# modular-ngp/phys-autodiff

Measured on NVIDIA B200. Metric: grid points/sec, fused MLP + finite-difference physics loss, higher is better.
Workload: dtype f32

## Files before the change

### phys_autodiff_b200/csrc/capi.cu

```cuda
#include "../../include/physad_b200.h"
#include "deep_data_kernels.cuh"
#include "deep_grad_kernels.cuh"
#include "deep_kernels.cuh"
#include "deep_tangent_kernels.cuh"
#include "deep_tc_kernels.cuh"
#include "dense_kernels.cuh"
#include "grad_kernels.cuh"
#include "stage_kernels.cuh"
#include "tangent_grad_kernels.cuh"
#include "tangent_kernels.cuh"

#include <algorithm>
#include <cmath>
#include <cstdio>
#include <cstdlib>
#include <cstring>
#include <string>
#include <unordered_map>
#include <vector>

using namespace physad;

namespace {

// ... 208 lines not shown
                    if (out) out->push_back(t * nzl + (nzl - rem));
                    continue;
                }
                const int take = std::max(1, std::min(rem, int(space)));
                cur += seg_cost + take;
                rem -= take;
                open = true;
                if (cur + seg_cost + 1.0 > cap) {
                    ++blocks; cur = 0.0; open = false;
                    if (out) out->push_back(t * nzl + (nzl - rem));
                }
            }
        }
        if (open) { ++blocks; if (out) out->push_back(tiles * nzl); }
        return blocks;
    };
    double lo = 1.0 + seg_cost, hi = double(tiles) * (nzl + seg_cost) + 1.0;
    for (int it = 0; it < 60; ++it) {
        const double mid = 0.5 * (lo + hi);
        if (fill(mid, nullptr) <= slots) hi = mid; else lo = mid;
    }
    std::vector<int> r;
    fill(hi, &r);
    return r;
}

int build_fused_plan(physad_ctx* c, const physad_grid* g, const physad_slab& s, int TX, int TY, long long slots,
                     cudaStream_t st) {
    if (int rc = ensure_coord_tables(c, g, st)) return rc;
    auto& p = c->plan;
    p.cxs = c->tab.dev;
    p.cys = p.cxs + g->nx;
    p.czs = p.cys + g->ny;
    const int key[10] = {g->nx, g->ny, g->nz, s.z_begin, s.z_end, c->cfg.norm, TX, TY, int(slots), 1};
    if (std::memcmp(key, p.key, sizeof(key)) == 0) return 0;
    const int tiles = ((g->nx + TX - 1) / TX) * ((g->ny + TY - 1) / TY), nzl = s.z_end - s.z_begin;
    const long long want = std::min<long long>(slots, (long long)tiles * nzl);
    const std::vector<int> ranges = balanced_ranges(tiles, nzl, want, 0.9);
    const size_t bytes = ranges.size() * sizeof(int);
    if (bytes > p.cap) {
        if (p.dev) CU(cudaFree(p.dev));
        p.dev = nullptr; p.cap = 0;
        CU(cudaMalloc(&p.dev, bytes));
        p.cap = bytes;
    }
    CU(cudaMemcpyAsync(p.dev, ranges.data(), bytes, cudaMemcpyHostToDevice, st));
    CU(cudaStreamSynchronize(st));
    p.ranges = reinterpret_cast<const int*>(p.dev);
    p.blocks = int(ranges.size()) - 1;
    std::memcpy(p.key, key, sizeof(key));
    return 0;
}

template <int H, int P, int TYB, int UNROLL, int MINB, bool PACKED, bool SPLITBAR, bool DPRES>
int launch_fused_d(physad_ctx* c, const physad_grid* g, const physad_slab& s, const float tc[3], bool xchg, double* acc,
                   float* const R[4], cudaStream_t st, int blocks_per_sm_cap = 0) {
    constexpr int TX = 32, TY = TYB * P;
    auto kern = k_fused_mlp_phys_loss<H, P, TYB, UNROLL, MINB, PACKED, SPLITBAR, DPRES>;
    const size_t smem = size_t(4) * 4 * (TX + 2) * (TY + 2) * sizeof(float);
    static const long long env_blocks = getenv("PHYSAD_FUSED_BLOCKS") ? atoll(getenv("PHYSAD_FUSED_BLOCKS")) : 0;
    int& per_sm = c->blocks_per_sm[reinterpret_cast<const void*>(kern)];
    if (per_sm == 0) {
        CU(cudaFuncSetAttribute(kern, cudaFuncAttributeMaxDynamicSharedMemorySize, int(smem)));
        int q = 0;
        CU(cudaOccupancyMaxActiveBlocksPerMultiprocessor(&q, kern, 32 * TYB, smem));
        if (q < 1) return fail(PHYSAD_E_UNSUPPORTED, "fused kernel does not fit on an SM");
        per_sm = q;
    }
    const int tiles_x = (g->nx + TX - 1) / TX, tiles_y = (g->ny + TY - 1) / TY;
    const int bps = blocks_per_sm_cap > 0 ? std::min(per_sm, blocks_per_sm_cap) : per_sm;
    const long long slots = env_blocks > 0 ? env_blocks : (long long)bps * c->sm_count;
    if (int rc = build_fused_plan(c, g, s, TX, TY, slots, st)) return rc;
    const long long blocks = c->plan.blocks;
    FusedArgs a{};
    a.nx = g->nx; a.ny = g->ny; a.nz = g->nz;
    a.z_begin = s.z_begin; a.z_end = s.z_end;
    a.tiles_x = tiles_x; a.tiles_y = tiles_y;
    a.cxs = c->plan.cxs; a.cys = c->plan.cys; a.czs = c->plan.czs; a.ranges = c->plan.ranges;
    a.m1p1 = c->cfg.norm == 1; a.periodic = g->periodic != 0;
    a.inv2dt = inv2(g->dt); a.inv2hx = inv2(g->hx); a.inv2hy = inv2(g->hy); a.inv2hz = inv2(g->hz);
    a.inv2dt_d = inv2d(g->dt); a.inv2hx_d = inv2d(g->hx); a.inv2hy_d = inv2d(g->hy); a.inv2hz_d = inv2d(g->hz);
    if (int rc = ensure_partials(c, size_t(blocks))) return rc;
    a.partials = c->partials; a.ticket = c->ticket; a.acc_out = acc;
    for (int k = 0; k < 4; ++k) a.R[k] = R[k];
    if (xchg) {
        a.x.rank = c->xrank; a.x.world = c->xworld; a.x.epoch = c->xepoch + 1;
        for (int p = 0; p < XCHG_MAX_RANKS; ++p) a.x.peer[p] = c->xpeer[p];
    }
    a.status = c->d_status;
    if (c->want_host_seq) { a.host_res = c->d_res; a.host_seq = c->want_host_seq; }
    if (c->trace && blocks <= c->trace_blocks) a.trace = c->trace;
    MlpConst<H> k;
    fill_const<H>(c, tc, k);
    kern<<<unsigned(blocks), 32 * TYB, smem, st>>>(k, a);
    CU(cudaGetLastError());
    c->launches++;
    if (xchg) c->xepoch++;
    return 0;
}

template <int H, int P, int TYB, int UNROLL, int MINB, bool PACKED, bool SPLITBAR = false>
int launch_fused_t(physad_ctx* c, const physad_grid* g, const physad_slab& s, const float tc[3], bool xchg, double* acc,
                   float* const R[4], cudaStream_t st, int blocks_per_sm_cap = 0) {
    return launch_fused_d<H, P, TYB, UNROLL, MINB, PACKED, SPLITBAR, false>(c, g, s, tc, xchg, acc, R, st, blocks_per_sm_cap);
}

template <int H, bool DPRES>
int launch_fused_default(physad_ctx* c, const physad_grid* g, const physad_slab& s, const float tc[3], bool xchg,
                         double* acc, float* const R[4], cudaStream_t st) {
    const long long tile_planes = (long long)((g->nx + 31) / 32) * ((g->ny + 63) / 64) * (s.z_end - s.z_begin);
    if (tile_planes < 12LL * c->sm_count)
        return launch_fused_d<H, 4, 8, 2, 2, true, true, DPRES>(c, g, s, tc, xchg, acc, R, st, 1);
    return launch_fused_d<H, 4, 16, 2, 1, true, true, DPRES>(c, g, s, tc, xchg, acc, R, st, 0);
}

template <int H>
int launch_fused_h(physad_ctx* c, const physad_grid* g, const physad_slab& s, const float tc[3], bool dt, double* acc,
                   float* const R[4], cudaStream_t st) {
    if (c->exact_residuals) return launch_fused_default<H, true>(c, g, s, tc, dt, acc, R, st);
    switch (c->fused_variant) {
        default:
        case 0: return launch_fused_default<H, false>(c, g, s, tc, dt, acc, R, st);
        case 1: return launch_fused_t<H, 4, 8, 2, 2, true, true>(c, g, s, tc, dt, acc, R, st);
        case 2: return launch_fused_t<H, 4, 16, 2, 1, true, false>(c, g, s, tc, dt, acc, R, st);
        case 3: return launch_fused_t<H, 4, 8, 2, 1, false, false>(c, g, s, tc, dt, acc, R, st);
        case 4: return launch_fused_t<H, 2, 16, 4, 1, true, true>(c, g, s, tc, dt, acc, R, st);
        case 5: return launch_fused_t<H, 1, 8, 4, 4, true, false>(c, g, s, tc, dt, acc, R, st);
        case 6: return launch_fused_t<H, 2, 8, 2, 3, true, true>(c, g, s, tc, dt, acc, R, st);
        case 7: return launch_fused_t<H, 4, 8, 2, 2, true, true>(c, g, s, tc, dt, acc, R, st, 1);
    }
}

int launch_fused(physad_ctx* c, const physad_grid* g, const physad_slab& s, float t, float dt, double* acc,
                 float* const R[4], cudaStream_t st, bool xchg = false) {
    if (c->advection != 0)
        return fail(PHYSAD_E_UNSUPPORTED, "fused_loss: the fused kernel implements the reference's central scheme only; "
                                          "upwind advection runs stage-wise (generate_fields + phys_loss)");
    if (xchg && (c->xworld <= 1 || !c->xbuf))
        return fail(PHYSAD_E_INVALID, "fused_loss_allreduce: call physad_xchg_connect first");
    if (s.z_end == s.z_begin) {
        XchgArgs x{};
        if (xchg) {
            x.rank = c->xrank; x.world = c->xworld; x.epoch = c->xepoch + 1;
            for (int p = 0; p < XCHG_MAX_RANKS; ++p) x.peer[p] = c->xpeer[p];
        }
        k_xchg_only<<<1, 32, 0, st>>>(x, acc, c->want_host_seq ? c->d_res : nullptr, c->want_host_seq, c->d_status);
        CU(cudaGetLastError());
        c->launches++;
        if (xchg) c->xepoch++;
        return 0;
    }
    const float ts[3] = {t - dt, t, t + dt};
    const float tc[3] = {time_coord(ts[0], c->cfg.norm), time_coord(ts[1], c->cfg.norm), time_coord(ts[2], c->cfg.norm)};
    switch (template_h(c->cfg.H)) {
        case 32: return launch_fused_h<32>(c, g, s, tc, xchg, acc, R, st);
        case 64: return launch_fused_h<64>(c, g, s, tc, xchg, acc, R, st);
        case 128: return launch_fused_h<128>(c, g, s, tc, xchg, acc, R, st);
    }
    return fail(PHYSAD_E_UNSUPPORTED, "H > 128 not built");
}

template <int H, bool FIELDS>
int launch_grid_t(physad_ctx* c, const physad_grid* g, const physad_slab& s, const float tc[3], GridInferArgs a,
                  cudaStream_t st, int dtype = PHYSAD_F32) {
    const int nzl = s.z_end - s.z_begin;
    if (nzl == 0) return 0;
// ... 1945 lines not shown
```

### phys_autodiff_b200/csrc/fused_loss.cuh

```cuda
#pragma once
#include <type_traits>

#include "mlp_eval.cuh"

namespace physad {

constexpr int XCHG_MAX_RANKS = 8;

struct XSlot {
    double a, b;
    unsigned long long flag;
    unsigned long long pad;
};

struct XchgArgs {
    int rank, world;
    unsigned long long epoch;
    XSlot* peer[XCHG_MAX_RANKS];
};

__device__ __forceinline__ void st_release_sys(unsigned long long* p, unsigned long long v) {
    asm volatile("st.release.sys.global.u64 [%0], %1;" ::"l"(p), "l"(v) : "memory");
}
__device__ __forceinline__ unsigned long long ld_acquire_sys(const unsigned long long* p) {
// ... 1 lines not shown
    asm volatile("ld.acquire.sys.global.u64 %0, [%1];" : "=l"(v) : "l"(p) : "memory");
    return v;
}
__device__ __forceinline__ double ld_relaxed_sys(const double* p) {
    double v;
    asm volatile("ld.relaxed.sys.global.f64 %0, [%1];" : "=d"(v) : "l"(p) : "memory");
    return v;
}

__device__ __forceinline__ bool xchg_allreduce2(const XchgArgs& x, double& a, double& b) {
    const int lane = threadIdx.x & 31;
    const int set = int(x.epoch & 1ull) * XCHG_MAX_RANKS;
    bool ok = true;
    double pa = 0.0, pb = 0.0;
    if (lane < x.world) {
        XSlot* s = x.peer[lane] + set + x.rank;
        s->a = a;
        s->b = b;
        __threadfence_system();
        st_release_sys(&s->flag, x.epoch);
        const XSlot* r = x.peer[x.rank] + set + lane;
        const long long t0 = clock64();
        while (ld_acquire_sys(&r->flag) != x.epoch) {
            if (clock64() - t0 > 8000000000ll) { ok = false; break; }
            __nanosleep(64);
        }
        pa = ld_relaxed_sys(&r->a);
        pb = ld_relaxed_sys(&r->b);
    }
    ok = __all_sync(0xffffffffu, ok);
    double ta = 0.0, tb = 0.0;
    for (int p = 0; p < x.world; ++p) {
        ta += __shfl_sync(0xffffffffu, pa, p);
        tb += __shfl_sync(0xffffffffu, pb, p);
    }
    a = ok ? ta : __longlong_as_double(0x7ff8000000000000ll);
    b = ok ? tb : __longlong_as_double(0x7ff8000000000000ll);
    return ok;
}

struct HostResult {
    double a, b;
    unsigned long long status;
    unsigned long long seq;
};

struct ReduceSink {
    const XchgArgs* x = nullptr;
    HostResult* host = nullptr;
    unsigned long long host_seq = 0;
    unsigned int* status = nullptr;
};

constexpr int TRACE_SLOTS = 18;
__device__ __forceinline__ unsigned long long globaltimer_ns() {
    unsigned long long t;
    asm volatile("mov.u64 %0, %%globaltimer;" : "=l"(t));
    return t;
}
__device__ __forceinline__ unsigned int smid() {
    unsigned int r;
    asm volatile("mov.u32 %0, %%smid;" : "=r"(r));
    return r;
}

struct FusedArgs {
    int nx, ny, nz;
    int z_begin, z_end;
    int tiles_x, tiles_y;
    const float* cxs;
    const float* cys;
    const float* czs;
    const int* ranges;
    int m1p1, periodic;
    float inv2dt, inv2hx, inv2hy, inv2hz;
    double inv2dt_d, inv2hx_d, inv2hy_d, inv2hz_d;
    double2* partials;
    unsigned int* ticket;
    double* acc_out;
    float* R[4];
    XchgArgs x;
    HostResult* host_res;
    unsigned long long host_seq;
    unsigned int* status;
    unsigned long long* trace;
};

__device__ __forceinline__ double warp_sum(double v) {
#pragma unroll
    for (int o = 16; o > 0; o >>= 1) v += __shfl_xor_sync(0xffffffffu, v, o);
    return v;
}

template <int NWARPS>
__device__ __forceinline__ void grid_reduce2_lin(double a, double b, double2* partials, unsigned int* ticket, double* out,
                                                 double2* s_red, unsigned int* s_flag, unsigned int block_lin,
                                                 unsigned int nblocks, const ReduceSink* sink = nullptr) {
    const int lane = threadIdx.x & 31, wid = threadIdx.x >> 5;
    a = warp_sum(a);
    b = warp_sum(b);
    if (lane == 0) s_red[wid] = make_double2(a, b);
    __syncthreads();
    if (threadIdx.x == 0) {
        double sa = 0.0, sb = 0.0;
#pragma unroll
        for (int i = 0; i < NWARPS; ++i) { sa += s_red[i].x; sb += s_red[i].y; }
        partials[block_lin] = make_double2(sa, sb);
// ... 23 lines not shown
            out[0] = ta;
            out[1] = tb;
            *ticket = 0u;
            if (sink != nullptr) {
                if (!ok && sink->status) *sink->status = 1u;
                if (sink->host) {
                    sink->host->a = ta;
                    sink->host->b = tb;
                    sink->host->status = ok ? 0ull : 1ull;
                    __threadfence_system();
                    st_release_sys(&sink->host->seq, sink->host_seq);
                }
            }
        }
    }
}

template <int NWARPS>
__device__ __forceinline__ void grid_reduce2(double a, double b, double2* partials, unsigned int* ticket, double* out,
                                             double2* s_red, unsigned int* s_flag, const ReduceSink* sink = nullptr) {
    grid_reduce2_lin<NWARPS>(a, b, partials, ticket, out, s_red, s_flag, blockIdx.x, gridDim.x, sink);
}

static __global__ void k_xchg_only(const __grid_constant__ XchgArgs x, double* out, HostResult* host, unsigned long long host_seq,
                            unsigned int* status) {
    double a = 0.0, b = 0.0;
    const bool ok = xchg_allreduce2(x, a, b);
    if (threadIdx.x == 0) {
        out[0] = a; out[1] = b;
        if (!ok && status) *status = 1u;
        if (host) {
            host->a = a; host->b = b; host->status = ok ? 0ull : 1ull;
            __threadfence_system();
            st_release_sys(&host->seq, host_seq);
        }
    }
}

__device__ __forceinline__ unsigned smem_u32(const void* p) { return unsigned(__cvta_generic_to_shared(p)); }
__device__ __forceinline__ void mbar_init(unsigned long long* bar, unsigned count) {
    asm volatile("mbarrier.init.shared::cta.b64 [%0], %1;" ::"r"(smem_u32(bar)), "r"(count) : "memory");
}
__device__ __forceinline__ void mbar_arrive(unsigned long long* bar) {
    asm volatile("{ .reg .b64 st; mbarrier.arrive.shared::cta.b64 st, [%0]; }" ::"r"(smem_u32(bar)) : "memory");
}
__device__ __forceinline__ void mbar_wait(unsigned long long* bar, unsigned parity) {
    unsigned ok;
    do {
        asm volatile("{ .reg .pred p; mbarrier.try_wait.parity.shared::cta.b64 p, [%1], %2; selp.u32 %0, 1, 0, p; }"
                     : "=r"(ok) : "r"(smem_u32(bar)), "r"(parity) : "memory");
    } while (!ok);
}

template <int H, int P, int TYB, int UNROLL, int MINB, bool PACKED, bool SPLITBAR = false, bool DPRES = false>
__global__ void __launch_bounds__(32 * TYB, MINB)
k_fused_mlp_phys_loss(const __grid_constant__ MlpConst<H> w, const FusedArgs a) {
    constexpr int TX = 32, TY = TYB * P, NWARPS = TYB;
    static_assert((NWARPS & (NWARPS - 1)) == 0, "warps per block must be a power of two");
    constexpr int SX = TX + 2, SY = TY + 2, CH = SX * SY, PLANE = 4 * CH, NB = 4;
    constexpr int RING = 2 * TX + 2 * TY, NTASK = (RING + 31) / 32;
    extern __shared__ float smem[];
    float* buf = smem;
    __shared__ double2 s_red[NWARPS];
    __shared__ unsigned int s_flag;
    __shared__ unsigned long long s_bar[2];
    auto stamp = [&](int slot) {
        if (a.trace != nullptr && threadIdx.x == 0) {
            unsigned long long* t = a.trace + (size_t(blockIdx.x) * TRACE_SLOTS + slot) * 2;
            t[0] = globaltimer_ns();
            t[1] = (unsigned long long)clock64();
        }
    };
    stamp(0);
    if (SPLITBAR) {
        if (threadIdx.x == 0) { mbar_init(&s_bar[0], NWARPS); mbar_init(&s_bar[1], NWARPS); }
        __syncthreads();
    }

    const int tx = threadIdx.x & 31, ty = threadIdx.x >> 5;
    const bool per = a.periodic != 0;

    const int nzl = a.z_end - a.z_begin;
    const long long W = (long long)a.tiles_x * a.tiles_y * nzl;
    (void)W;
    const long long w_end = a.ranges[blockIdx.x + 1];
    long long wpos = a.ranges[blockIdx.x];
    double acc_s = 0.0, acc_u = 0.0;
    int kbuf = 0;
    int seg = 0;
    if (a.trace != nullptr && threadIdx.x == 0) {
        unsigned long long* t = a.trace + (size_t(blockIdx.x) * TRACE_SLOTS + 15) * 2;
        t[0] = smid();
        t[1] = (unsigned long long)(w_end - wpos);
    }
    stamp(1);

  while (wpos < w_end) {
    const int tile = int(wpos / nzl);
    const int zs = int(wpos - (long long)tile * nzl);
    const int nplanes = int(w_end - wpos < (long long)(nzl - zs) ? w_end - wpos : (long long)(nzl - zs));
    wpos += nplanes;
    const int zc0 = a.z_begin + zs;
    const int x0 = (tile % a.tiles_x) * TX, y0 = (tile / a.tiles_x) * TY;

    const int gx = x0 + tx;
    const float cx = __ldg(a.cxs + bc_index(gx, a.nx, per));
    float cy[P];
    bool live[P];
#pragma unroll
    for (int j = 0; j < P; ++j) {
        const int gy = y0 + ty + j * TYB;
        cy[j] = __ldg(a.cys + bc_index(gy, a.ny, per));
        live[j] = gx < a.nx && gy < a.ny;
    }
    using real = typename std::conditional<DPRES, double, float>::type;
    const real i2t = DPRES ? real(a.inv2dt_d) : real(a.inv2dt), i2x = DPRES ? real(a.inv2hx_d) : real(a.inv2hx);
    const real i2y = DPRES ? real(a.inv2hy_d) : real(a.inv2hy), i2z = DPRES ? real(a.inv2hz_d) : real(a.inv2hz);
    real dT[P][4];
#pragma unroll
    for (int j = 0; j < P; ++j)
#pragma unroll
        for (int c = 0; c < 4; ++c) dT[j][c] = real(0);

    if (seg < 4) stamp(2 + 3 * seg);
    float cz_next = __ldg(a.czs + bc_index(zc0 - 1, a.nz, per));
    for (int k = 0; k <= nplanes + 1; ++k, ++kbuf) {
        const int zk = zc0 - 1 + k;
        const float cz = cz_next;
        cz_next = __ldg(a.czs + bc_index(zk + 1, a.nz, per));
        if (k == 1 && seg < 4) stamp(3 + 3 * seg);
        float* pl = buf + (kbuf & (NB - 1)) * PLANE;
        const bool halo_plane = (k == 0) || (k == nplanes + 1);
        real dTn[P][4];
        if (halo_plane) {
            float y[P][1][4];
            mlp_eval<H, 1, P, UNROLL, PACKED>(w, cx, cy, cz, y);
#pragma unroll
            for (int j = 0; j < P; ++j) {
                const int o = (1 + ty + j * TYB) * SX + 1 + tx;
#pragma unroll
                for (int c = 0; c < 4; ++c) { pl[c * CH + o] = y[j][0][c]; dTn[j][c] = real(0); }
            }
        } else {
            float y[P][3][4];
            mlp_eval<H, 3, P, UNROLL, PACKED>(w, cx, cy, cz, y);
#pragma unroll
            for (int j = 0; j < P; ++j) {
                const int o = (1 + ty + j * TYB) * SX + 1 + tx;
#pragma unroll
                for (int c = 0; c < 4; ++c) {
                    pl[c * CH + o] = y[j][1][c];
                    dTn[j][c] = central_diff(y[j][2][c], y[j][0][c], i2t);
                }
            }
            {
                static_assert(NTASK <= NWARPS, "one ring task per warp and plane");
                const int i = (ty - kbuf) & (NWARPS - 1);
                if (i < NTASK) {
                    const int r = i * 32 + tx;
                    int xx, yy;
                    if (r < TX) { xx = 1 + r; yy = 0; }
                    else if (r < 2 * TX) { xx = 1 + r - TX; yy = SY - 1; }
                    else if (r < 2 * TX + TY) { xx = 0; yy = 1 + r - 2 * TX; }
                    else { xx = SX - 1; yy = 1 + r - 2 * TX - TY; }
                    if (r >= RING) { xx = 0; yy = 0; }
                    const float rcx = __ldg(a.cxs + bc_index(x0 - 1 + xx, a.nx, per));
                    const float rc[1] = {__ldg(a.cys + bc_index(y0 - 1 + yy, a.ny, per))};
                    float yr[1][1][4];
                    mlp_eval<H, 1, 1, UNROLL, PACKED>(w, rcx, rc, cz, yr);
                    if (r < RING) {
#pragma unroll
                        for (int c = 0; c < 4; ++c) pl[c * CH + yy * SX + xx] = yr[0][0][c];
                    }
                }
            }
        }
        if (SPLITBAR) {
            __syncwarp();
            if (tx == 0) mbar_arrive(&s_bar[kbuf & 1]);
            if (kbuf >= 1) mbar_wait(&s_bar[(kbuf - 1) & 1], unsigned((kbuf - 1) >> 1) & 1u);
        } else {
            __syncthreads();
        }
        if (k >= 2) {
            const float* pc = buf + ((kbuf - 1) & (NB - 1)) * PLANE;
            const float* pm = buf + ((kbuf - 2) & (NB - 1)) * PLANE;
            const float* pp = pl;
            const int zl = zk - 1 - a.z_begin;
#pragma unroll
            for (int j = 0; j < P; ++j) {
                const int o = (1 + ty + j * TYB) * SX + 1 + tx;
                float f[4], R[4];
                real gxv[4], gyv[4], gzv[4];
#pragma unroll
                for (int c = 0; c < 4; ++c) {
                    const float* q = pc + c * CH + o;
                    f[c] = q[0];
                    gxv[c] = central_diff(q[1], q[-1], i2x);
                    gyv[c] = central_diff(q[SX], q[-SX], i2y);
                    gzv[c] = central_diff(pp[c * CH + o], pm[c * CH + o], i2z);
                }
                point_residual(f, gxv, gyv, gzv, dT[j], R);
                const float Rs = R[0], Rx = R[1], Ry = R[2], Rz = R[3];
                if (live[j]) {
                    acc_s += double(Rs) * double(Rs);
                    acc_u += double(Rx) * double(Rx) + double(Ry) * double(Ry) + double(Rz) * double(Rz);
                    if (a.R[0]) {
                        const size_t i = (size_t(zl) * a.ny + (y0 + ty + j * TYB)) * a.nx + gx;
                        a.R[0][i] = Rs; a.R[1][i] = Rx; a.R[2][i] = Ry; a.R[3][i] = Rz;
                    }
                }
            }
        }
#pragma unroll
        for (int j = 0; j < P; ++j)
#pragma unroll
            for (int c = 0; c < 4; ++c) dT[j][c] = dTn[j][c];
    }
    if (!SPLITBAR) __syncthreads();
    if (seg < 4) stamp(4 + 3 * seg);
    ++seg;
  }
    stamp(14);
    ReduceSink sink;
    sink.x = &a.x; sink.host = a.host_res; sink.host_seq = a.host_seq; sink.status = a.status;
    grid_reduce2<NWARPS>(acc_s, acc_u, a.partials, a.ticket, a.acc_out, s_red, &s_flag, &sink);
    stamp(16);
}

}
```

### phys_autodiff_b200/csrc/mlp_eval.cuh

```cuda
#pragma once
#include <cuda_runtime.h>

namespace physad {

template <int H>
struct MlpConst {
    static_assert(H % 2 == 0, "hidden units are processed in pairs");
    float2 b1p[H / 2];
    float2 w0s[H / 2];
    float2 w1s[H / 2];
    float2 w2s[H / 2];
    float2 ptm[H / 2];
    float2 pt0[H / 2];
    float2 ptp[H / 2];
    float4 w2[H];
    float4 b2;
};

__device__ __forceinline__ float relu_ref(float s) {
    return fmaxf(s, 0.f);
}

__device__ __forceinline__ float axis_coord(int i, int n, bool m1p1) {
    if (n <= 1) return 0.f;
    const float u = __fdiv_rn(float(i), float(n - 1));
    return m1p1 ? __fsub_rn(__fmul_rn(2.f, u), 1.f) : u;
}

__device__ __forceinline__ int bc_index(int v, int n, bool periodic) {
    if (periodic) {
        int r = v % n;
        return r < 0 ? r + n : r;
    }
    return v < 0 ? 0 : (v > n - 1 ? n - 1 : v);
}

typedef unsigned long long f32x2;

__device__ __forceinline__ f32x2 pack2(float lo, float hi) {
    f32x2 r;
    asm("mov.b64 %0, {%1, %2};" : "=l"(r) : "f"(lo), "f"(hi));
    return r;
}
__device__ __forceinline__ void unpack2(f32x2 v, float& lo, float& hi) {
    asm("mov.b64 {%0, %1}, %2;" : "=f"(lo), "=f"(hi) : "l"(v));
}
__device__ __forceinline__ f32x2 mul2_rn(f32x2 a, f32x2 b) {
    f32x2 r;
    asm("mul.rn.f32x2 %0, %1, %2;" : "=l"(r) : "l"(a), "l"(b));
    return r;
}
__device__ __forceinline__ f32x2 add2_rn_swapped(f32x2 acc, f32x2 p) {
    float lo, hi;
    unpack2(p, lo, hi);
    f32x2 r;
    asm("add.rn.f32x2 %0, %1, %2;" : "=l"(r) : "l"(acc), "l"(pack2(hi, lo)));
    return r;
}

__device__ __forceinline__ f32x2 add2_rn(f32x2 a, f32x2 b) {
    f32x2 r;
    asm("add.rn.f32x2 %0, %1, %2;" : "=l"(r) : "l"(a), "l"(b));
    return r;
}
__device__ __forceinline__ f32x2 pack2(float2 v) { return pack2(v.x, v.y); }
__device__ __forceinline__ f32x2 bcast2(float v) { return pack2(v, v); }

template <int H, int NS, int P, int UNROLL, bool PACKED>
__device__ __forceinline__ void mlp_eval(const MlpConst<H>& w, float cx, const float (&cy)[P], float cz,
                                         float (&y)[P][NS][4]) {
    const float4 b2 = w.b2;
    f32x2 q01[P][NS], q23[P][NS];
#pragma unroll
    for (int j = 0; j < P; ++j)
#pragma unroll
        for (int s = 0; s < NS; ++s) {
            if (PACKED) {
                q01[j][s] = pack2(b2.x, b2.y);
                q23[j][s] = pack2(b2.z, b2.w);
            } else {
                y[j][s][0] = b2.x; y[j][s][1] = b2.y; y[j][s][2] = b2.z; y[j][s][3] = b2.w;
            }
        }
#pragma unroll UNROLL
    for (int q = 0; q < H / 2; ++q) {
        const float2 b1p = w.b1p[q], w0s = w.w0s[q], w1s = w.w1s[q], w2s = w.w2s[q];
        const float2 tm = w.ptm[q], t0 = w.pt0[q], tp = w.ptp[q];
        const float4 ca = w.w2[2 * q], cb = w.w2[2 * q + 1];
        if (PACKED) {
            const f32x2 sx = add2_rn_swapped(pack2(b1p), mul2_rn(pack2(w0s), bcast2(cx)));
            const f32x2 mz = mul2_rn(pack2(w2s), bcast2(cz));
            const f32x2 ca10 = pack2(ca.x, ca.y), ca32 = pack2(ca.z, ca.w);
            const f32x2 cb10 = pack2(cb.x, cb.y), cb32 = pack2(cb.z, cb.w);
#pragma unroll
            for (int j = 0; j < P; ++j) {
                const f32x2 sxy = add2_rn_swapped(sx, mul2_rn(pack2(w1s), bcast2(cy[j])));
                const f32x2 sxyz = add2_rn_swapped(sxy, mz);
#pragma unroll
                for (int s = 0; s < NS; ++s) {
                    const float2 pt = (NS == 1) ? t0 : (s == 0 ? tm : (s == 1 ? t0 : tp));
                    float v0, v1;
                    unpack2(add2_rn(sxyz, pack2(pt)), v0, v1);
                    const f32x2 a0 = bcast2(relu_ref(v0)), a1 = bcast2(relu_ref(v1));
                    q01[j][s] = add2_rn_swapped(q01[j][s], mul2_rn(a0, ca10));
                    q23[j][s] = add2_rn_swapped(q23[j][s], mul2_rn(a0, ca32));
                    q01[j][s] = add2_rn_swapped(q01[j][s], mul2_rn(a1, cb10));
                    q23[j][s] = add2_rn_swapped(q23[j][s], mul2_rn(a1, cb32));
                }
            }
        } else {
#pragma unroll
            for (int e = 0; e < 2; ++e) {
                const float b1 = e ? b1p.y : b1p.x, w0 = e ? w0s.x : w0s.y, w1 = e ? w1s.x : w1s.y, w2 = e ? w2s.x : w2s.y;
                const float4 c = e ? cb : ca;
                const float sx = __fadd_rn(b1, __fmul_rn(w0, cx));
                const float mz = __fmul_rn(w2, cz);
#pragma unroll
                for (int j = 0; j < P; ++j) {
                    const float sxyz = __fadd_rn(__fadd_rn(sx, __fmul_rn(w1, cy[j])), mz);
#pragma unroll
                    for (int s = 0; s < NS; ++s) {
                        const float2 pt2 = (NS == 1) ? t0 : (s == 0 ? tm : (s == 1 ? t0 : tp));
                        const float act = relu_ref(__fadd_rn(sxyz, e ? pt2.y : pt2.x));
                        y[j][s][0] = __fadd_rn(y[j][s][0], __fmul_rn(c.y, act));
                        y[j][s][1] = __fadd_rn(y[j][s][1], __fmul_rn(c.x, act));
                        y[j][s][2] = __fadd_rn(y[j][s][2], __fmul_rn(c.w, act));
                        y[j][s][3] = __fadd_rn(y[j][s][3], __fmul_rn(c.z, act));
                    }
                }
            }
        }
    }
    if (PACKED) {
#pragma unroll
        for (int j = 0; j < P; ++j)
#pragma unroll
            for (int s = 0; s < NS; ++s) {
                unpack2(q01[j][s], y[j][s][0], y[j][s][1]);
                unpack2(q23[j][s], y[j][s][2], y[j][s][3]);
            }
    }
}

__device__ __forceinline__ float central_diff(float plus, float minus, float inv2h) {
    return __fmul_rn(__fsub_rn(plus, minus), inv2h);
}
__device__ __forceinline__ double central_diff(float plus, float minus, double inv2h) {
    return __dmul_rn(__dsub_rn(double(plus), double(minus)), inv2h);
}

__device__ __forceinline__ void point_residual(const float (&f)[4], const float (&gx)[4], const float (&gy)[4],
                                               const float (&gz)[4], const float (&dT)[4], float (&R)[4]) {
    const float div = __fadd_rn(__fadd_rn(gx[1], gy[2]), gz[3]);
#pragma unroll
    for (int c = 0; c < 4; ++c) {
        const float adv = __fmaf_rn(f[3], gz[c], __fmaf_rn(f[2], gy[c], __fmul_rn(f[1], gx[c])));
        R[c] = __fadd_rn(dT[c], adv);
    }
    R[0] = __fmaf_rn(f[0], div, R[0]);
}

__device__ __forceinline__ void point_residual(const float (&f)[4], const double (&gx)[4], const double (&gy)[4],
                                               const double (&gz)[4], const double (&dT)[4], float (&R)[4]) {
    const double ux = double(f[1]), uy = double(f[2]), uz = double(f[3]);
    const double div = __dadd_rn(__dadd_rn(gx[1], gy[2]), gz[3]);
#pragma unroll
    for (int c = 0; c < 4; ++c) {
        const double adv = __dadd_rn(__dadd_rn(__dmul_rn(ux, gx[c]), __dmul_rn(uy, gy[c])), __dmul_rn(uz, gz[c]));
        const double r = __dadd_rn(dT[c], adv);
        R[c] = float(c == 0 ? __dadd_rn(r, __dmul_rn(double(f[0]), div)) : r);
    }
}

template <typename T>
__device__ __forceinline__ void point_residual_upwind(const float (&f)[4], const float (&xm)[4], const float (&xp)[4],
                                                      const float (&ym)[4], const float (&yp)[4], const float (&zm)[4],
                                                      const float (&zp)[4], const T (&dT)[4], T i1x, T i1y, T i1z, T i2x, T i2y,
                                                      T i2z, float (&R)[4]) {
    const T div = ((T(xp[1]) - T(xm[1])) * i2x + (T(yp[2]) - T(ym[2])) * i2y) + (T(zp[3]) - T(zm[3])) * i2z;
#pragma unroll
    for (int c = 0; c < 4; ++c) {
        const T ax = f[1] > 0.f ? (T(f[c]) - T(xm[c])) * i1x : (T(xp[c]) - T(f[c])) * i1x;
        const T ay = f[2] > 0.f ? (T(f[c]) - T(ym[c])) * i1y : (T(yp[c]) - T(f[c])) * i1y;
        const T az = f[3] > 0.f ? (T(f[c]) - T(zm[c])) * i1z : (T(zp[c]) - T(f[c])) * i1z;
        T r = dT[c] + ((T(f[1]) * ax + T(f[2]) * ay) + T(f[3]) * az);
        if (c == 0) r += T(f[0]) * div;
        R[c] = float(r);
    }
}

}
```

### phys_autodiff_b200/ops.py

```python
from __future__ import annotations

import ctypes as C
from typing import Optional, Sequence

import numpy as np

from . import capi
from .capi import Grid, MLPConfig, PhysWeights, CSlab, check, ptr


def slab_for_rank(nz: int, rank: int, world: int) -> tuple[int, int]:
    return (rank * nz) // world, ((rank + 1) * nz) // world


def _f32(a) -> np.ndarray:
    return np.ascontiguousarray(a, dtype=np.float32)


class Context:

    def __init__(self, device: Optional[int] = None):
        self._lib = capi.lib()
        self._h = C.c_void_p()
        check(self._lib.physad_ctx_create(C.byref(self._h), C.c_int(-1 if device is None else device)), "ctx_create")
# ... 12 lines not shown
        except Exception:
            pass

    @property
    def sm_count(self) -> int:
        return int(self._lib.physad_ctx_sm_count(self._h))

    @property
    def launch_count(self) -> int:
        return int(self._lib.physad_launch_count(self._h))

    def set_exact_residuals(self, on: bool) -> bool:
        return bool(self._lib.physad_set_exact_residuals(self._h, C.c_int(int(on))))

    def set_advection(self, upwind: bool) -> bool:
        return bool(self._lib.physad_set_advection(self._h, C.c_int(int(upwind))))

    def set_fused_variant(self, v: int) -> int:
        return int(self._lib.physad_set_fused_variant(self._h, C.c_int(v)))

    def connect_peers(self, group=None) -> bool:
        import torch
        import torch.distributed as dist
        if not dist.is_initialized() or dist.get_world_size(group) == 1:
            return False
        world, rank = dist.get_world_size(group), dist.get_rank(group)
        buf = C.create_string_buffer(64)
        ok = self._lib.physad_xchg_export(self._h, buf) == 0
        handles = [None] * world
        dist.all_gather_object(handles, bytes(buf.raw) if ok else None, group=group)
        if ok and all(h is not None for h in handles):
            blob = C.create_string_buffer(b"".join(handles), 64 * world)
            ok = self._lib.physad_xchg_connect(self._h, C.c_int(rank), C.c_int(world), blob) == 0
        else:
            ok = False
        flag = torch.tensor([1 if ok else 0], device="cuda")
        dist.all_reduce(flag, op=dist.ReduceOp.MIN, group=group)
        if not bool(flag.item()):
            self._lib.physad_xchg_disconnect(self._h)
            self._peers = None
            return False
        self._peers = (rank, world)
        return True

    def xchg_status(self) -> bool:
        v = C.c_int(0)
        check(self._lib.physad_xchg_status(self._h, C.byref(v)), "xchg_status")
        return bool(v.value)

    def set_fused_trace(self, buf=None) -> None:
        if buf is None:
            check(self._lib.physad_set_fused_trace(self._h, None, C.c_int(0)), "set_fused_trace")
        else:
            check(self._lib.physad_set_fused_trace(self._h, ptr(buf), C.c_int(buf.numel() // 36)), "set_fused_trace")
        self._trace_keep = buf

    def disconnect_peers(self) -> None:
        self._lib.physad_xchg_disconnect(self._h)
        self._peers = None

    def set_weights(self, cfg: MLPConfig, W1, b1, W2, b2) -> None:
        W1, b1, W2, b2 = _f32(W1), _f32(b1), _f32(W2), _f32(b2)
        assert W1.size == cfg.H * cfg.In and b1.size == cfg.H and W2.size == cfg.Out * cfg.H and b2.size == cfg.Out
        c = cfg.c()
        check(self._lib.physad_set_weights(self._h, C.byref(c), ptr(W1), ptr(b1), ptr(W2), ptr(b2)), "set_weights")
        self.cfg = cfg
        self.hidden_layers = None

    @staticmethod
    def _stream():
        import torch
        return C.c_void_p(torch.cuda.current_stream().cuda_stream)

    @staticmethod
    def _slab(g: Grid, slab):
        z0, z1 = (0, g.nz) if slab is None else slab
        return CSlab(z0, z1), (z1 - z0) * g.ny * g.nx

    @staticmethod
    def _empty(n, dtype=None):
        import torch
        return torch.empty(n, dtype=dtype or torch.float32, device="cuda")

    def mlp_forward(self, x):
        B = x.shape[0]
        y = self._empty(B * self.cfg.Out)
        check(self._lib.physad_mlp_forward_dev(self._h, ptr(x), ptr(y), C.c_size_t(B), self._stream()), "mlp_forward")
        return y.view(B, self.cfg.Out)

    def mlp_grid_infer(self, g: Grid, t: float, slab=None):
        cs, n = self._slab(g, slab)
        out = self._empty(n * 4)
        cg = g.c()
        check(self._lib.physad_mlp_grid_infer_dev(self._h, C.byref(cg), C.byref(cs), C.c_float(t), ptr(out),
                                                  self._stream()), "mlp_grid_infer")
        return out.view(n, 4)

    def mlp_generate_fields(self, g: Grid, t: float, dt: float, slab=None):
        cs, n = self._slab(g, slab)
        s = [self._empty(n) for _ in range(3)]
        u = [self._empty(3 * n) for _ in range(3)]
        cg = g.c()
        check(self._lib.physad_mlp_generate_fields_dev(self._h, C.byref(cg), C.byref(cs), C.c_float(t), C.c_float(dt),
                                                       ptr(s[0]), ptr(s[1]), ptr(s[2]), ptr(u[0]), ptr(u[1]), ptr(u[2]),
                                                       self._stream()), "mlp_generate_fields")
        return s[0], s[1], s[2], u[0], u[1], u[2]

# ... 725 lines not shown
```

Measured before the change: 15.74 billion.

## Precompute per-tile first-layer x/y terms into shared memory tables

For the packed path, each block now precomputes the first-layer x contribution (bias plus w0*x) and y contribution (w1*y) for every hidden pair and every tile column/row, including halo, into shared memory. The MLP evaluation then reads these from the tables instead of recomputing them from coordinates, and the ring halo evaluation no longer reloads coordinates from global memory. This trades recomputed multiplies and global loads for extra shared memory, which can lower occupancy, plus an upfront fill loop and a barrier per tile. The end-of-segment barrier is also made unconditional under SPLITBAR.

```diff
diff --git a/phys_autodiff_b200/csrc/capi.cu b/phys_autodiff_b200/csrc/capi.cu
--- a/phys_autodiff_b200/csrc/capi.cu
+++ b/phys_autodiff_b200/csrc/capi.cu
@@ -289,7 +289,8 @@
                    float* const R[4], cudaStream_t st, int blocks_per_sm_cap = 0) {
     constexpr int TX = 32, TY = TYB * P;
     auto kern = k_fused_mlp_phys_loss<H, P, TYB, UNROLL, MINB, PACKED, SPLITBAR, DPRES>;
-    const size_t smem = size_t(4) * 4 * (TX + 2) * (TY + 2) * sizeof(float);
+    const size_t smem = size_t(4) * 4 * (TX + 2) * (TY + 2) * sizeof(float) +
+                        (PACKED ? size_t(H / 2) * ((TX + 2) + (TY + 2)) * sizeof(float2) : 0);
     static const long long env_blocks = getenv("PHYSAD_FUSED_BLOCKS") ? atoll(getenv("PHYSAD_FUSED_BLOCKS")) : 0;
     int& per_sm = c->blocks_per_sm[reinterpret_cast<const void*>(kern)];
     if (per_sm == 0) {
diff --git a/phys_autodiff_b200/csrc/fused_loss.cuh b/phys_autodiff_b200/csrc/fused_loss.cuh
--- a/phys_autodiff_b200/csrc/fused_loss.cuh
+++ b/phys_autodiff_b200/csrc/fused_loss.cuh
@@ -207,6 +207,29 @@
     } while (!ok);
 }
 
+template <int SY, int P, int TYB>
+__device__ __forceinline__ int yt_slot(int yy) {
+    return yy == 0 ? 0 : (yy == SY - 1 ? 1 : 2 + ((yy - 1) % TYB) * P + (yy - 1) / TYB);
+}
+
+template <int SX, int SY, int P>
+struct L1FromTables {
+    static_assert(SY % 2 == 0, "16-byte aligned yt rows");
+    const float2* xt;
+    const float2* yt;
+    template <int H>
+    __device__ __forceinline__ f32x2 x_term(const MlpConst<H>&, int) const { return pack2(*xt); }
+    __device__ __forceinline__ void next() { xt += SX; yt += SY; }
+    template <int H>
+    __device__ __forceinline__ f32x2 y_term(const MlpConst<H>&, int, int j) const {
+        if (P % 2 == 0) {
+            const float4 v = reinterpret_cast<const float4*>(yt)[j / 2];
+            return (j & 1) ? pack2(v.z, v.w) : pack2(v.x, v.y);
+        }
+        return pack2(yt[j]);
+    }
+};
+
 template <int H, int P, int TYB, int UNROLL, int MINB, bool PACKED, bool SPLITBAR = false, bool DPRES = false>
 __global__ void __launch_bounds__(32 * TYB, MINB)
 k_fused_mlp_phys_loss(const __grid_constant__ MlpConst<H> w, const FusedArgs a) {
@@ -214,8 +237,10 @@
     static_assert((NWARPS & (NWARPS - 1)) == 0, "warps per block must be a power of two");
     constexpr int SX = TX + 2, SY = TY + 2, CH = SX * SY, PLANE = 4 * CH, NB = 4;
     constexpr int RING = 2 * TX + 2 * TY, NTASK = (RING + 31) / 32;
-    extern __shared__ float smem[];
+    extern __shared__ __align__(16) float smem[];
     float* buf = smem;
+    float2* xt = reinterpret_cast<float2*>(buf + NB * PLANE);
+    float2* yt = xt + (H / 2) * SX;
     __shared__ double2 s_red[NWARPS];
     __shared__ unsigned int s_flag;
     __shared__ unsigned long long s_bar[2];
@@ -278,6 +303,20 @@
         for (int c = 0; c < 4; ++c) dT[j][c] = real(0);
 
     if (seg < 4) stamp(2 + 3 * seg);
+    if (PACKED) {
+        for (int i = threadIdx.x; i < (H / 2) * (SX + SY); i += 32 * NWARPS) {
+            const int q = i / (SX + SY), c = i - q * (SX + SY);
+            const bool is_x = c < SX;
+            const float v = is_x ? __ldg(a.cxs + bc_index(x0 - 1 + c, a.nx, per))
+                                 : __ldg(a.cys + bc_index(y0 - 1 + (c - SX), a.ny, per));
+            const float vy[1] = {v};
+            const L1FromCoords<1> l1{v, vy};
+            float2 t;
+            unpack2(is_x ? l1.x_term(w, q) : l1.y_term(w, q, 0), t.x, t.y);
+            (is_x ? xt + q * SX + c : yt + q * SY + yt_slot<SY, P, TYB>(c - SX))[0] = t;
+        }
+        __syncthreads();
+    }
     float cz_next = __ldg(a.czs + bc_index(zc0 - 1, a.nz, per));
     for (int k = 0; k <= nplanes + 1; ++k, ++kbuf) {
         const int zk = zc0 - 1 + k;
@@ -289,7 +328,8 @@
         real dTn[P][4];
         if (halo_plane) {
             float y[P][1][4];
-            mlp_eval<H, 1, P, UNROLL, PACKED>(w, cx, cy, cz, y);
+            if (PACKED) mlp_eval_packed<H, 1, P, UNROLL>(w, L1FromTables<SX, SY, P>{xt + 1 + tx, yt + 2 + ty * P}, cz, y);
+            else mlp_eval<H, 1, P, UNROLL, false>(w, cx, cy, cz, y);
 #pragma unroll
             for (int j = 0; j < P; ++j) {
                 const int o = (1 + ty + j * TYB) * SX + 1 + tx;
@@ -298,7 +338,8 @@
             }
         } else {
             float y[P][3][4];
-            mlp_eval<H, 3, P, UNROLL, PACKED>(w, cx, cy, cz, y);
+            if (PACKED) mlp_eval_packed<H, 3, P, UNROLL>(w, L1FromTables<SX, SY, P>{xt + 1 + tx, yt + 2 + ty * P}, cz, y);
+            else mlp_eval<H, 3, P, UNROLL, false>(w, cx, cy, cz, y);
 #pragma unroll
             for (int j = 0; j < P; ++j) {
                 const int o = (1 + ty + j * TYB) * SX + 1 + tx;
@@ -319,10 +360,14 @@
                     else if (r < 2 * TX + TY) { xx = 0; yy = 1 + r - 2 * TX; }
                     else { xx = SX - 1; yy = 1 + r - 2 * TX - TY; }
                     if (r >= RING) { xx = 0; yy = 0; }
-                    const float rcx = __ldg(a.cxs + bc_index(x0 - 1 + xx, a.nx, per));
-                    const float rc[1] = {__ldg(a.cys + bc_index(y0 - 1 + yy, a.ny, per))};
                     float yr[1][1][4];
-                    mlp_eval<H, 1, 1, UNROLL, PACKED>(w, rcx, rc, cz, yr);
+                    if (PACKED) {
+                        mlp_eval_packed<H, 1, 1, UNROLL>(w, L1FromTables<SX, SY, 1>{xt + xx, yt + yt_slot<SY, P, TYB>(yy)}, cz, yr);
+                    } else {
+                        const float rcx = __ldg(a.cxs + bc_index(x0 - 1 + xx, a.nx, per));
+                        const float rc[1] = {__ldg(a.cys + bc_index(y0 - 1 + yy, a.ny, per))};
+                        mlp_eval<H, 1, 1, UNROLL, false>(w, rcx, rc, cz, yr);
+                    }
                     if (r < RING) {
 #pragma unroll
                         for (int c = 0; c < 4; ++c) pl[c * CH + yy * SX + xx] = yr[0][0][c];
@@ -372,7 +417,7 @@
 #pragma unroll
             for (int c = 0; c < 4; ++c) dT[j][c] = dTn[j][c];
     }
-    if (!SPLITBAR) __syncthreads();
+    __syncthreads();
     if (seg < 4) stamp(4 + 3 * seg);
     ++seg;
   }
diff --git a/phys_autodiff_b200/csrc/mlp_eval.cuh b/phys_autodiff_b200/csrc/mlp_eval.cuh
--- a/phys_autodiff_b200/csrc/mlp_eval.cuh
+++ b/phys_autodiff_b200/csrc/mlp_eval.cuh
@@ -66,79 +66,107 @@
 __device__ __forceinline__ f32x2 pack2(float2 v) { return pack2(v.x, v.y); }
 __device__ __forceinline__ f32x2 bcast2(float v) { return pack2(v, v); }
 
+template <int P>
+struct L1FromCoords {
+    float cx;
+    const float (&cy)[P];
+    template <int H>
+    __device__ __forceinline__ f32x2 x_term(const MlpConst<H>& w, int q) const {
+        return add2_rn_swapped(pack2(w.b1p[q]), mul2_rn(pack2(w.w0s[q]), bcast2(cx)));
+    }
+    template <int H>
+    __device__ __forceinline__ f32x2 y_term(const MlpConst<H>& w, int q, int j) const {
+        return mul2_rn(pack2(w.w1s[q]), bcast2(cy[j]));
+    }
+    __device__ __forceinline__ void next() {}
+};
+
+template <int H, int NS, int P, int UNROLL, class L1>
+__device__ __forceinline__ void mlp_eval_packed(const MlpConst<H>& w, L1 l1, float cz, float (&y)[P][NS][4]) {
+    const float4 b2 = w.b2;
+    f32x2 q01[P][NS], q23[P][NS];
+#pragma unroll
+    for (int j = 0; j < P; ++j)
+#pragma unroll
+        for (int s = 0; s < NS; ++s) {
+            q01[j][s] = pack2(b2.x, b2.y);
+            q23[j][s] = pack2(b2.z, b2.w);
+        }
+#pragma unroll UNROLL
+    for (int q = 0; q < H / 2; ++q) {
+        const f32x2 sx = l1.x_term(w, q);
+        const float2 w2s = w.w2s[q];
+        const float2 tm = w.ptm[q], t0 = w.pt0[q], tp = w.ptp[q];
+        const float4 ca = w.w2[2 * q], cb = w.w2[2 * q + 1];
+        const f32x2 mz = mul2_rn(pack2(w2s), bcast2(cz));
+        const f32x2 ca10 = pack2(ca.x, ca.y), ca32 = pack2(ca.z, ca.w);
+        const f32x2 cb10 = pack2(cb.x, cb.y), cb32 = pack2(cb.z, cb.w);
+#pragma unroll
+        for (int j = 0; j < P; ++j) {
+            const f32x2 sxy = add2_rn_swapped(sx, l1.y_term(w, q, j));
+            const f32x2 sxyz = add2_rn_swapped(sxy, mz);
+#pragma unroll
+            for (int s = 0; s < NS; ++s) {
+                const float2 pt = (NS == 1) ? t0 : (s == 0 ? tm : (s == 1 ? t0 : tp));
+                float v0, v1;
+                unpack2(add2_rn(sxyz, pack2(pt)), v0, v1);
+                const f32x2 a0 = bcast2(relu_ref(v0)), a1 = bcast2(relu_ref(v1));
+                q01[j][s] = add2_rn_swapped(q01[j][s], mul2_rn(a0, ca10));
+                q23[j][s] = add2_rn_swapped(q23[j][s], mul2_rn(a0, ca32));
+                q01[j][s] = add2_rn_swapped(q01[j][s], mul2_rn(a1, cb10));
+                q23[j][s] = add2_rn_swapped(q23[j][s], mul2_rn(a1, cb32));
+            }
+        }
+        l1.next();
+    }
+#pragma unroll
+    for (int j = 0; j < P; ++j)
+#pragma unroll
+        for (int s = 0; s < NS; ++s) {
+            unpack2(q01[j][s], y[j][s][0], y[j][s][1]);
+            unpack2(q23[j][s], y[j][s][2], y[j][s][3]);
+        }
+}
+
 template <int H, int NS, int P, int UNROLL, bool PACKED>
 __device__ __forceinline__ void mlp_eval(const MlpConst<H>& w, float cx, const float (&cy)[P], float cz,
                                          float (&y)[P][NS][4]) {
+    if (PACKED) {
+        mlp_eval_packed<H, NS, P, UNROLL>(w, L1FromCoords<P>{cx, cy}, cz, y);
+        return;
+    }
     const float4 b2 = w.b2;
-    f32x2 q01[P][NS], q23[P][NS];
 #pragma unroll
     for (int j = 0; j < P; ++j)
 #pragma unroll
         for (int s = 0; s < NS; ++s) {
-            if (PACKED) {
-                q01[j][s] = pack2(b2.x, b2.y);
-                q23[j][s] = pack2(b2.z, b2.w);
-            } else {
-                y[j][s][0] = b2.x; y[j][s][1] = b2.y; y[j][s][2] = b2.z; y[j][s][3] = b2.w;
-            }
+            y[j][s][0] = b2.x; y[j][s][1] = b2.y; y[j][s][2] = b2.z; y[j][s][3] = b2.w;
         }
 #pragma unroll UNROLL
     for (int q = 0; q < H / 2; ++q) {
         const float2 b1p = w.b1p[q], w0s = w.w0s[q], w1s = w.w1s[q], w2s = w.w2s[q];
         const float2 tm = w.ptm[q], t0 = w.pt0[q], tp = w.ptp[q];
         const float4 ca = w.w2[2 * q], cb = w.w2[2 * q + 1];
-        if (PACKED) {
-            const f32x2 sx = add2_rn_swapped(pack2(b1p), mul2_rn(pack2(w0s), bcast2(cx)));
-            const f32x2 mz = mul2_rn(pack2(w2s), bcast2(cz));
-            const f32x2 ca10 = pack2(ca.x, ca.y), ca32 = pack2(ca.z, ca.w);
-            const f32x2 cb10 = pack2(cb.x, cb.y), cb32 = pack2(cb.z, cb.w);
+#pragma unroll
+        for (int e = 0; e < 2; ++e) {
+            const float b1 = e ? b1p.y : b1p.x, w0 = e ? w0s.x : w0s.y, w1 = e ? w1s.x : w1s.y, w2 = e ? w2s.x : w2s.y;
+            const float4 c = e ? cb : ca;
+            const float sx = __fadd_rn(b1, __fmul_rn(w0, cx));
+            const float mz = __fmul_rn(w2, cz);
 #pragma unroll
             for (int j = 0; j < P; ++j) {
-                const f32x2 sxy = add2_rn_swapped(sx, mul2_rn(pack2(w1s), bcast2(cy[j])));
-                const f32x2 sxyz = add2_rn_swapped(sxy, mz);
+                const float sxyz = __fadd_rn(__fadd_rn(sx, __fmul_rn(w1, cy[j])), mz);
 #pragma unroll
                 for (int s = 0; s < NS; ++s) {
-                    const float2 pt = (NS == 1) ? t0 : (s == 0 ? tm : (s == 1 ? t0 : tp));
-                    float v0, v1;
-                    unpack2(add2_rn(sxyz, pack2(pt)), v0, v1);
-                    const f32x2 a0 = bcast2(relu_ref(v0)), a1 = bcast2(relu_ref(v1));
-                    q01[j][s] = add2_rn_swapped(q01[j][s], mul2_rn(a0, ca10));
-                    q23[j][s] = add2_rn_swapped(q23[j][s], mul2_rn(a0, ca32));
-                    q01[j][s] = add2_rn_swapped(q01[j][s], mul2_rn(a1, cb10));
-                    q23[j][s] = add2_rn_swapped(q23[j][s], mul2_rn(a1, cb32));
+                    const float2 pt2 = (NS == 1) ? t0 : (s == 0 ? tm : (s == 1 ? t0 : tp));
+                    const float act = relu_ref(__fadd_rn(sxyz, e ? pt2.y : pt2.x));
+                    y[j][s][0] = __fadd_rn(y[j][s][0], __fmul_rn(c.y, act));
+                    y[j][s][1] = __fadd_rn(y[j][s][1], __fmul_rn(c.x, act));
+                    y[j][s][2] = __fadd_rn(y[j][s][2], __fmul_rn(c.w, act));
+                    y[j][s][3] = __fadd_rn(y[j][s][3], __fmul_rn(c.z, act));
                 }
             }
-        } else {
-#pragma unroll
-            for (int e = 0; e < 2; ++e) {
-                const float b1 = e ? b1p.y : b1p.x, w0 = e ? w0s.x : w0s.y, w1 = e ? w1s.x : w1s.y, w2 = e ? w2s.x : w2s.y;
-                const float4 c = e ? cb : ca;
-                const float sx = __fadd_rn(b1, __fmul_rn(w0, cx));
-                const float mz = __fmul_rn(w2, cz);
-#pragma unroll
-                for (int j = 0; j < P; ++j) {
-                    const float sxyz = __fadd_rn(__fadd_rn(sx, __fmul_rn(w1, cy[j])), mz);
-#pragma unroll
-                    for (int s = 0; s < NS; ++s) {
-                        const float2 pt2 = (NS == 1) ? t0 : (s == 0 ? tm : (s == 1 ? t0 : tp));
-                        const float act = relu_ref(__fadd_rn(sxyz, e ? pt2.y : pt2.x));
-                        y[j][s][0] = __fadd_rn(y[j][s][0], __fmul_rn(c.y, act));
-                        y[j][s][1] = __fadd_rn(y[j][s][1], __fmul_rn(c.x, act));
-                        y[j][s][2] = __fadd_rn(y[j][s][2], __fmul_rn(c.w, act));
-                        y[j][s][3] = __fadd_rn(y[j][s][3], __fmul_rn(c.z, act));
-                    }
-                }
-            }
-        }
-    }
-    if (PACKED) {
-#pragma unroll
-        for (int j = 0; j < P; ++j)
-#pragma unroll
-            for (int s = 0; s < NS; ++s) {
-                unpack2(q01[j][s], y[j][s][0], y[j][s][1]);
-                unpack2(q23[j][s], y[j][s][2], y[j][s][3]);
-            }
+        }
     }
 }
 
```

Result: faster. 16.22 billion (median of 6 runs) (+3.0%).

## Interleave shared-memory plane channels as float4 and add per-warp phase tracing

Applied to the files above, without the earlier changes.

Changes the shared-memory plane buffer from four channel-planar float arrays to one interleaved float4 per grid point. Each store and each stencil neighbour read becomes a single 128-bit shared access instead of four scalar ones, which cuts the number of shared load/store instructions in the stencil. It also adds an optional trace variant that records per-warp clock() cycles for each phase, chosen only when tracing is enabled. The risk is more bank conflicts on the wide shared accesses, and the larger trace buffer layout changes the Python-side slot size.

```diff
diff --git a/phys_autodiff_b200/csrc/capi.cu b/phys_autodiff_b200/csrc/capi.cu
--- a/phys_autodiff_b200/csrc/capi.cu
+++ b/phys_autodiff_b200/csrc/capi.cu
@@ -284,11 +284,11 @@
     return 0;
 }
 
-template <int H, int P, int TYB, int UNROLL, int MINB, bool PACKED, bool SPLITBAR, bool DPRES>
+template <int H, int P, int TYB, int UNROLL, int MINB, bool PACKED, bool SPLITBAR, bool DPRES, bool TRACE = false>
 int launch_fused_d(physad_ctx* c, const physad_grid* g, const physad_slab& s, const float tc[3], bool xchg, double* acc,
                    float* const R[4], cudaStream_t st, int blocks_per_sm_cap = 0) {
     constexpr int TX = 32, TY = TYB * P;
-    auto kern = k_fused_mlp_phys_loss<H, P, TYB, UNROLL, MINB, PACKED, SPLITBAR, DPRES>;
+    auto kern = k_fused_mlp_phys_loss<H, P, TYB, UNROLL, MINB, PACKED, SPLITBAR, DPRES, TRACE>;
     const size_t smem = size_t(4) * 4 * (TX + 2) * (TY + 2) * sizeof(float);
     static const long long env_blocks = getenv("PHYSAD_FUSED_BLOCKS") ? atoll(getenv("PHYSAD_FUSED_BLOCKS")) : 0;
     int& per_sm = c->blocks_per_sm[reinterpret_cast<const void*>(kern)];
@@ -337,13 +337,15 @@
     return launch_fused_d<H, P, TYB, UNROLL, MINB, PACKED, SPLITBAR, false>(c, g, s, tc, xchg, acc, R, st, blocks_per_sm_cap);
 }
 
-template <int H, bool DPRES>
+template <int H, bool DPRES, bool TRACE = false>
 int launch_fused_default(physad_ctx* c, const physad_grid* g, const physad_slab& s, const float tc[3], bool xchg,
                          double* acc, float* const R[4], cudaStream_t st) {
+    if constexpr (!DPRES && !TRACE)
+        if (c->trace) return launch_fused_default<H, false, true>(c, g, s, tc, xchg, acc, R, st);
     const long long tile_planes = (long long)((g->nx + 31) / 32) * ((g->ny + 63) / 64) * (s.z_end - s.z_begin);
     if (tile_planes < 12LL * c->sm_count)
-        return launch_fused_d<H, 4, 8, 2, 2, true, true, DPRES>(c, g, s, tc, xchg, acc, R, st, 1);
-    return launch_fused_d<H, 4, 16, 2, 1, true, true, DPRES>(c, g, s, tc, xchg, acc, R, st, 0);
+        return launch_fused_d<H, 4, 8, 2, 2, true, true, DPRES, TRACE>(c, g, s, tc, xchg, acc, R, st, 1);
+    return launch_fused_d<H, 4, 16, 2, 1, true, true, DPRES, TRACE>(c, g, s, tc, xchg, acc, R, st, 0);
 }
 
 template <int H>
diff --git a/phys_autodiff_b200/csrc/fused_loss.cuh b/phys_autodiff_b200/csrc/fused_loss.cuh
--- a/phys_autodiff_b200/csrc/fused_loss.cuh
+++ b/phys_autodiff_b200/csrc/fused_loss.cuh
@@ -77,7 +77,9 @@
     unsigned int* status = nullptr;
 };
 
-constexpr int TRACE_SLOTS = 18;
+constexpr int TRACE_WARPS = 16, TRACE_PHASES = 6;
+constexpr int TRACE_SLOTS = 18 + TRACE_WARPS * TRACE_PHASES / 2;
+enum TracePhase { PH_EVAL = 0, PH_RING, PH_WAIT, PH_STENCIL, PH_HALO, PH_LAST };
 __device__ __forceinline__ unsigned long long globaltimer_ns() {
     unsigned long long t;
     asm volatile("mov.u64 %0, %%globaltimer;" : "=l"(t));
@@ -207,15 +209,15 @@
     } while (!ok);
 }
 
-template <int H, int P, int TYB, int UNROLL, int MINB, bool PACKED, bool SPLITBAR = false, bool DPRES = false>
+template <int H, int P, int TYB, int UNROLL, int MINB, bool PACKED, bool SPLITBAR = false, bool DPRES = false, bool TRACE = false>
 __global__ void __launch_bounds__(32 * TYB, MINB)
 k_fused_mlp_phys_loss(const __grid_constant__ MlpConst<H> w, const FusedArgs a) {
     constexpr int TX = 32, TY = TYB * P, NWARPS = TYB;
     static_assert((NWARPS & (NWARPS - 1)) == 0, "warps per block must be a power of two");
-    constexpr int SX = TX + 2, SY = TY + 2, CH = SX * SY, PLANE = 4 * CH, NB = 4;
+    constexpr int SX = TX + 2, SY = TY + 2, PLANE = SX * SY, NB = 4;
     constexpr int RING = 2 * TX + 2 * TY, NTASK = (RING + 31) / 32;
-    extern __shared__ float smem[];
-    float* buf = smem;
+    extern __shared__ float4 smem4[];
+    float4* buf = smem4;
     __shared__ double2 s_red[NWARPS];
     __shared__ unsigned int s_flag;
     __shared__ unsigned long long s_bar[2];
@@ -227,6 +229,22 @@
         }
     };
     stamp(0);
+    static_assert(!TRACE || NWARPS <= TRACE_WARPS, "phase trace slots");
+    __shared__ unsigned int s_ph[TRACE ? NWARPS : 1][TRACE_PHASES];
+    auto lap = [&](int ph) {
+        if (TRACE) {
+            unsigned int t;
+            asm volatile("mov.u32 %0, %%tid.x;" : "=r"(t));
+            if ((t & 31u) == 0u) {
+                unsigned int* row = s_ph[t >> 5];
+                const unsigned int now = unsigned(clock());
+                if (ph >= 0) row[ph] += now - row[PH_LAST];
+                row[PH_LAST] = now;
+            }
+        }
+    };
+    if (TRACE && (threadIdx.x & 31) == 0)
+        for (int p = 0; p < TRACE_PHASES; ++p) s_ph[threadIdx.x >> 5][p] = 0u;
     if (SPLITBAR) {
         if (threadIdx.x == 0) { mbar_init(&s_bar[0], NWARPS); mbar_init(&s_bar[1], NWARPS); }
         __syncthreads();
@@ -279,12 +297,13 @@
 
     if (seg < 4) stamp(2 + 3 * seg);
     float cz_next = __ldg(a.czs + bc_index(zc0 - 1, a.nz, per));
+    lap(-1);
     for (int k = 0; k <= nplanes + 1; ++k, ++kbuf) {
         const int zk = zc0 - 1 + k;
         const float cz = cz_next;
         cz_next = __ldg(a.czs + bc_index(zk + 1, a.nz, per));
         if (k == 1 && seg < 4) stamp(3 + 3 * seg);
-        float* pl = buf + (kbuf & (NB - 1)) * PLANE;
+        float4* pl = buf + (kbuf & (NB - 1)) * PLANE;
         const bool halo_plane = (k == 0) || (k == nplanes + 1);
         real dTn[P][4];
         if (halo_plane) {
@@ -294,8 +313,10 @@
             for (int j = 0; j < P; ++j) {
                 const int o = (1 + ty + j * TYB) * SX + 1 + tx;
 #pragma unroll
-                for (int c = 0; c < 4; ++c) { pl[c * CH + o] = y[j][0][c]; dTn[j][c] = real(0); }
-            }
+                for (int c = 0; c < 4; ++c) dTn[j][c] = real(0);
+                pl[o] = make_float4(y[j][0][0], y[j][0][1], y[j][0][2], y[j][0][3]);
+            }
+            lap(PH_HALO);
         } else {
             float y[P][3][4];
             mlp_eval<H, 3, P, UNROLL, PACKED>(w, cx, cy, cz, y);
@@ -304,10 +325,11 @@
                 const int o = (1 + ty + j * TYB) * SX + 1 + tx;
 #pragma unroll
                 for (int c = 0; c < 4; ++c) {
-                    pl[c * CH + o] = y[j][1][c];
                     dTn[j][c] = central_diff(y[j][2][c], y[j][0][c], i2t);
                 }
-            }
+                pl[o] = make_float4(y[j][1][0], y[j][1][1], y[j][1][2], y[j][1][3]);
+            }
+            lap(PH_EVAL);
             {
                 static_assert(NTASK <= NWARPS, "one ring task per warp and plane");
                 const int i = (ty - kbuf) & (NWARPS - 1);
@@ -325,10 +347,11 @@
                     mlp_eval<H, 1, 1, UNROLL, PACKED>(w, rcx, rc, cz, yr);
                     if (r < RING) {
 #pragma unroll
-                        for (int c = 0; c < 4; ++c) pl[c * CH + yy * SX + xx] = yr[0][0][c];
+                        pl[yy * SX + xx] = make_float4(yr[0][0][0], yr[0][0][1], yr[0][0][2], yr[0][0][3]);
                     }
                 }
             }
+            lap(PH_RING);
         }
         if (SPLITBAR) {
             __syncwarp();
@@ -337,23 +360,26 @@
         } else {
             __syncthreads();
         }
+        lap(PH_WAIT);
         if (k >= 2) {
-            const float* pc = buf + ((kbuf - 1) & (NB - 1)) * PLANE;
-            const float* pm = buf + ((kbuf - 2) & (NB - 1)) * PLANE;
-            const float* pp = pl;
+            const float4* pc = buf + ((kbuf - 1) & (NB - 1)) * PLANE;
+            const float4* pm = buf + ((kbuf - 2) & (NB - 1)) * PLANE;
+            const float4* pp = pl;
             const int zl = zk - 1 - a.z_begin;
 #pragma unroll
             for (int j = 0; j < P; ++j) {
                 const int o = (1 + ty + j * TYB) * SX + 1 + tx;
                 float f[4], R[4];
                 real gxv[4], gyv[4], gzv[4];
+                const float4 v0 = pc[o], vxm = pc[o - 1], vxp = pc[o + 1], vym = pc[o - SX], vyp = pc[o + SX];
+                const float4 vzm = pm[o], vzp = pp[o];
+                auto ch = [](const float4& v, int c) { return c == 0 ? v.x : (c == 1 ? v.y : (c == 2 ? v.z : v.w)); };
 #pragma unroll
                 for (int c = 0; c < 4; ++c) {
-                    const float* q = pc + c * CH + o;
-                    f[c] = q[0];
-                    gxv[c] = central_diff(q[1], q[-1], i2x);
-                    gyv[c] = central_diff(q[SX], q[-SX], i2y);
-                    gzv[c] = central_diff(pp[c * CH + o], pm[c * CH + o], i2z);
+                    f[c] = ch(v0, c);
+                    gxv[c] = central_diff(ch(vxp, c), ch(vxm, c), i2x);
+                    gyv[c] = central_diff(ch(vyp, c), ch(vym, c), i2y);
+                    gzv[c] = central_diff(ch(vzp, c), ch(vzm, c), i2z);
                 }
                 point_residual(f, gxv, gyv, gzv, dT[j], R);
                 const float Rs = R[0], Rx = R[1], Ry = R[2], Rz = R[3];
@@ -366,6 +392,7 @@
                     }
                 }
             }
+            lap(PH_STENCIL);
         }
 #pragma unroll
         for (int j = 0; j < P; ++j)
@@ -377,6 +404,9 @@
     ++seg;
   }
     stamp(14);
+    if (TRACE && a.trace != nullptr && tx == 0)
+        for (int p = 0; p < TRACE_PHASES; ++p)
+            a.trace[(size_t(blockIdx.x) * TRACE_SLOTS + 18) * 2 + ty * TRACE_PHASES + p] = s_ph[ty][p];
     ReduceSink sink;
     sink.x = &a.x; sink.host = a.host_res; sink.host_seq = a.host_seq; sink.status = a.status;
     grid_reduce2<NWARPS>(acc_s, acc_u, a.partials, a.ticket, a.acc_out, s_red, &s_flag, &sink);
diff --git a/phys_autodiff_b200/ops.py b/phys_autodiff_b200/ops.py
--- a/phys_autodiff_b200/ops.py
+++ b/phys_autodiff_b200/ops.py
@@ -88,7 +88,7 @@
         if buf is None:
             check(self._lib.physad_set_fused_trace(self._h, None, C.c_int(0)), "set_fused_trace")
         else:
-            check(self._lib.physad_set_fused_trace(self._h, ptr(buf), C.c_int(buf.numel() // 36)), "set_fused_trace")
+            check(self._lib.physad_set_fused_trace(self._h, ptr(buf), C.c_int(buf.numel() // 132)), "set_fused_trace")
         self._trace_keep = buf
 
     def disconnect_peers(self) -> None:
```

Result: no change. 15.75 billion before, 15.61 billion after (median of 6 runs) (-0.9%).
